# antoyang/FrozenBiLM

Hardware: AMD Instinct MI355X
Metric: video-text samples/sec (MLM fwd+bwd) DeBERTa-XL+adapters (higher is better)
Workload: dtype bf16; 1 GPU; DeBERTa-v2-XLarge(24L)+adapters ds8/8, B=32/GPU, T=10x1024, L=256 (S=266), MLM fwd+bwd+allreduce+clip+Adam, dropout 0.1 live, seeded random weights; global_batch=32, seq_len=266, parallelism=dp1, dead_layer23_encoder_pass=skipped (output unused, SURVEY fact 6); FLOPs still counted

## Files before the change

frozenbilm_amd/bert_engine.py:

```python
from __future__ import annotations

import math
from dataclasses import dataclass
from typing import Dict, List, Optional

import torch

from . import lib as L
from .engine import BF16, F32, Engine, NormRef, Packing, Run, Stream, _ru, _StepFn


@dataclass
class BertLayerSave:
    qkv: torch.Tensor
    ctx: torch.Tensor
    lse: torch.Tensor
    gp: torch.Tensor
    ln1: NormRef
    ln2: NormRef
    seed_att: int
    seed_ln1: int
    seed_ln2: int


# ... 25 lines not shown
    offs = [0]
    for v in plen_h:
        offs.append(offs[-1] + v)
    row0 = torch.tensor(offs, dtype=torch.int32, device=dev)
    b_of = torch.repeat_interleave(torch.arange(B, device=dev), torch.tensor(plen_h, device=dev), output_size=n)
    pos = torch.arange(n, device=dev) - row0[:-1].long()[b_of]
    sel = b_of * S + pos
    inv = torch.full((B * S,), -1, dtype=torch.int64, device=dev)
    inv[sel] = torch.arange(n, device=dev)
    return Packing(row0=row0, sel=sel, inv=inv, pos=pos, n=n)


class BertEngine:
    _ln = Engine._ln
    _ln_bwd = Engine._ln_bwd
    _materialize = Engine._materialize
    attach_grads = Engine.attach_grads

    def __init__(self, model):
        self.m = model
        cfg = model.config
        self.cfg = cfg
        self.H, self.I, self.V = cfg.hidden_size, cfg.intermediate_size, cfg.vocab_size
        self.nh, self.nL = cfg.num_attention_heads, cfg.num_hidden_layers
        if self.H != 64 * self.nh or self.H % 64 or self.I % 64:
            raise NotImplementedError(f"the fused attention takes head_dim 64 (hidden {self.H}, {self.nh} heads) and the GEMMs "
                                      "need hidden / intermediate sizes that are multiples of 64")
        self.F = model.features_dim
        self.Fp = _ru(self.F, 64) if self.F else 0
        self.Vp = _ru(self.V, 64)
# ... 403 lines not shown
```

frozenbilm_amd/build.py:

```python
from __future__ import annotations

import concurrent.futures as cf
import os
import shutil
import subprocess
import sys

HERE = os.path.dirname(os.path.abspath(__file__))
CSRC = os.path.join(HERE, "csrc")
DEBUG = os.environ.get("FBL_DEBUG_BUILD", "0") == "1"
OBJ = os.path.join(HERE, "csrc", "build_dbg" if DEBUG else "build")
LIB = os.path.join(HERE, "libfbl_dbg.so" if DEBUG else "libfbl.so")
ARCH = "gfx950"
FLAGS = ["--offload-arch=" + ARCH, "-O3", "-std=c++17", "-fPIC", "-fno-gpu-rdc", "-Wno-unused-result"]
if DEBUG:
    FLAGS.append("-DFBL_DEBUG_SWITCHES")
    FLAGS += os.environ.get("FBL_DEBUG_EXTRA_FLAGS", "").split()
    if os.environ.get("FBL_DEBUG_LIB_NAME"):
        LIB = os.path.join(HERE, os.environ["FBL_DEBUG_LIB_NAME"])
        OBJ = os.path.join(HERE, "csrc", "build_dbg_" + os.path.splitext(os.environ["FBL_DEBUG_LIB_NAME"])[0])


def _hipcc() -> str:
    for cand in (os.environ.get("HIPCC"), shutil.which("hipcc"), "/opt/rocm/bin/hipcc"):
        if cand and os.path.exists(cand):
            return cand
    raise RuntimeError("hipcc not found (need ROCm >= 7.0 with gfx950 support)")


def sources():
    return sorted(os.path.join(CSRC, f) for f in os.listdir(CSRC) if f.endswith(".hip"))


def _deps_mtime() -> float:
    hdrs = [os.path.join(CSRC, f) for f in os.listdir(CSRC) if f.endswith(".h")]
    hdrs += [os.path.join(os.path.dirname(HERE), "include", h) for h in ("fbl.h", "fbl_mha.h")]
    return max(os.path.getmtime(h) for h in hdrs)


def _compile(src: str, force: bool) -> str:
    obj = os.path.join(OBJ, os.path.basename(src)[:-4] + ".o")
    if not force and os.path.exists(obj) and os.path.getmtime(obj) > max(os.path.getmtime(src), _deps_mtime()):
        return obj
    cmd = [_hipcc(), *FLAGS, "-Rpass-analysis=kernel-resource-usage", "-c", src, "-o", obj]
    r = subprocess.run(cmd, capture_output=True, text=True)
    if r.returncode != 0:
        raise RuntimeError(f"hipcc failed for {src}:\n{r.stdout}\n{r.stderr}")
    bad, name = [], "?"
    for line in r.stderr.splitlines():
        if "Function Name:" in line:
            name = line.split("Function Name:")[1].split("[")[0].strip()
# ... 33 lines not shown
```

frozenbilm_amd/csrc/rowops.hip:

```cpp
#include "fbl_common.h"
#include "../../include/fbl.h"

namespace {

template <int VEC>
struct VecF {};
template <>
struct VecF<4> {
  typedef f32x4 T;
};
template <>
struct VecF<2> {
  typedef f32x2 T;
};

template <int VEC>
__device__ __forceinline__ void ldf(const float* p, float* v) {
  if (VEC == 4) {
    f32x4 x = *(const f32x4*)p;
    v[0] = x[0]; v[1] = x[1]; v[2] = x[2]; v[3] = x[3];
  } else if (VEC == 2) {
    f32x2 x = *(const f32x2*)p;
    v[0] = x[0]; v[1] = x[1];
  } else {
// ... 11 lines not shown
  if (VEC == 4) *(bf16x4*)p = (bf16x4){f2bf(v[0]), f2bf(v[1]), f2bf(v[2]), f2bf(v[3])};
  else if (VEC == 2) *(bf16x2*)p = (bf16x2){f2bf(v[0]), f2bf(v[1])};
  else p[0] = f2bf(v[0]);
}

struct LnFwdArgs {
  const float* y; long ldy; float p_drop; uint64_t seed; const uint64_t* seed_dev;
  const float* r_plain; const float* r_t; const float* r_stats; const float* r_gamma; const float* r_beta;
  const int32_t* r_rowmask;
  const float* gamma; const float* beta; float eps; const int32_t* rowmask;
  float* out_t; float* out_stats; bf16* out_bf16; float* out_f32;
  int N, H;
};

template <int EPL>
__global__ __launch_bounds__(256) void ln_fwd_kernel(LnFwdArgs a) {
  constexpr int VEC = (EPL % 4 == 0) ? 4 : ((EPL % 2 == 0) ? 2 : 1);
  constexpr int NIT = EPL / VEC;
  const int lane = threadIdx.x & 63;
  const int row = blockIdx.x * 4 + (threadIdx.x >> 6);
  if (row >= a.N) return;
  const int H = a.H;
  float v[EPL];
  const uint32_t thr = fbl_drop_thresh(a.p_drop);
  const float inv_keep = a.p_drop > 0.f ? 1.0f / (1.0f - a.p_drop) : 1.0f;
  const uint64_t seed = a.p_drop > 0.f ? fbl_seed(a.seed, a.seed_dev) : 0;
  float rmean = 0.f, rrstd = 0.f, rmask = 1.f;
  if (a.r_t) {
    rmean = a.r_stats[2 * (long)row];
    rrstd = a.r_stats[2 * (long)row + 1];
    if (a.r_rowmask) rmask = (float)a.r_rowmask[row];
  }
#pragma unroll
  for (int it = 0; it < NIT; ++it) {
    const int col = (it * 64 + lane) * VEC;
    float* vv = v + it * VEC;
// ... 38 lines not shown
  if (lane == 0 && a.out_stats) {
    a.out_stats[2 * (long)row] = mean;
    a.out_stats[2 * (long)row + 1] = rstd;
  }
  const float om = a.rowmask ? (float)a.rowmask[row] : 1.0f;
#pragma unroll
  for (int it = 0; it < NIT; ++it) {
    const int col = (it * 64 + lane) * VEC;
    float gg[VEC], bb[VEC], o[VEC];
    ldf<VEC>(a.gamma + col, gg);
    ldf<VEC>(a.beta + col, bb);
#pragma unroll
    for (int c = 0; c < VEC; ++c) o[c] = ((v[it * VEC + c] - mean) * rstd * gg[c] + bb[c]) * om;
    if (a.out_bf16) stb<VEC>(a.out_bf16 + (long)row * H + col, o);
    if (a.out_f32) stf<VEC>(a.out_f32 + (long)row * H + col, o);
  }
}

struct LnMatArgs {
  const float* t; const float* stats; const float* gamma; const float* beta; const int32_t* rowmask;
  const float* add_bcast; int S; float* out_f32; bf16* out_bf16; int N, H;
};
template <int EPL>
__global__ __launch_bounds__(256) void ln_mat_kernel(LnMatArgs a) {
  constexpr int VEC = (EPL % 4 == 0) ? 4 : ((EPL % 2 == 0) ? 2 : 1);
  constexpr int NIT = EPL / VEC;
  const int lane = threadIdx.x & 63;
  const int row = blockIdx.x * 4 + (threadIdx.x >> 6);
  if (row >= a.N) return;
  const int H = a.H;
// ... 711 lines not shown
  return 0;
}

extern "C" int fbl_ln_materialize(const float* t, const float* stats, const float* gamma, const float* beta,
                                  const int32_t* rowmask, const float* add_bcast, int S, float* out_f32, void* out_bf16,
                                  int N, int H, void* stream) {
  if (H % 64 || H > 2048) return FBL_ERR_SHAPE;
  if (N <= 0) return 0;
  LnMatArgs a{t, stats, gamma, beta, rowmask, add_bcast, S > 0 ? S : 1, out_f32, (bf16*)out_bf16, N, H};
  dim3 grid((N + 3) / 4);
  FBL_EPL_DISPATCH(H, ln_mat_kernel, grid, a, (hipStream_t)stream);
  FBL_CHECK_LAUNCH();
  return 0;
}

extern "C" int64_t fbl_ln_bwd_ws_floats(int H) { return (int64_t)LNB_BLOCKS * 3 * H; }
extern "C" int fbl_ln_bwd(const float* dout, const int32_t* rowmask, const float* t, const float* stats,
                          const float* gamma, float p_drop, uint64_t seed, const uint64_t* seed_dev, float* out_dt, void* out_dy_bf16,
                          float* out_dy_f32, float* dgamma, float* dbeta, float* dysum, float* ws, int N, int H,
                          int64_t ld_dy_bf16, void* stream) {
  if (H % 64 || H > 2048) return FBL_ERR_SHAPE;
  if (N <= 0) return 0;
  if (ld_dy_bf16 == 0) ld_dy_bf16 = H;
  if (ld_dy_bf16 < H || (ld_dy_bf16 % 8)) return FBL_ERR_ALIGN;
  LnBwdArgs a{dout, rowmask, t, stats, gamma, p_drop, seed, seed_dev, out_dt, (bf16*)out_dy_bf16, out_dy_f32, ws, N, H, ld_dy_bf16};
  int nblk;
  if ((H / 64) % 2 == 0) {
    nblk = (N + 1) / 2;
    if (nblk > LNB_BLOCKS) nblk = LNB_BLOCKS;
    dim3 grid(nblk);
    switch (H / 64) {
      case 2: hipLaunchKernelGGL(ln_bwd2_kernel<2>, grid, dim3(256), 0, (hipStream_t)stream, a); break;
      case 4: hipLaunchKernelGGL(ln_bwd2_kernel<4>, grid, dim3(256), 0, (hipStream_t)stream, a); break;
      case 8: hipLaunchKernelGGL(ln_bwd2_kernel<8>, grid, dim3(256), 0, (hipStream_t)stream, a); break;
      case 12: hipLaunchKernelGGL(ln_bwd2_kernel<12>, grid, dim3(256), 0, (hipStream_t)stream, a); break;
      case 16: hipLaunchKernelGGL(ln_bwd2_kernel<16>, grid, dim3(256), 0, (hipStream_t)stream, a); break;
      case 24: hipLaunchKernelGGL(ln_bwd2_kernel<24>, grid, dim3(256), 0, (hipStream_t)stream, a); break;
      case 32: hipLaunchKernelGGL(ln_bwd2_kernel<32>, grid, dim3(256), 0, (hipStream_t)stream, a); break;
      default: return FBL_ERR_SHAPE;
    }
  } else {
    nblk = (N + 3) / 4;
    if (nblk > LNB_BLOCKS) nblk = LNB_BLOCKS;
    dim3 grid(nblk);
    FBL_EPL_DISPATCH(H, ln_bwd_kernel, grid, a, (hipStream_t)stream);
  }
  FBL_CHECK_LAUNCH();
  if (dgamma || dbeta || dysum) {
    hipLaunchKernelGGL(ln_bwd_fold_kernel, dim3((3 * H + 31) / 32), dim3(256), 0, (hipStream_t)stream, ws, nblk, H,
                       dgamma, dbeta, dysum);
    FBL_CHECK_LAUNCH();
  }
  return 0;
}

extern "C" int fbl_im2col3(const void* x_bf16, void* out_bf16, int B, int S, int H, void* stream) {
  if (H % 8) return FBL_ERR_SHAPE;
  if (B * S <= 0) return 0;
  hipLaunchKernelGGL(im2col3_kernel, dim3(B * S), dim3(256), 0, (hipStream_t)stream, (const bf16*)x_bf16,
                     (bf16*)out_bf16, B, S, H);
  FBL_CHECK_LAUNCH();
  return 0;
}
extern "C" int fbl_col2im3(const float* dcol, float* dx, int B, int S, int H, int accumulate, void* stream) {
  if (H % 4) return FBL_ERR_SHAPE;
  if (B * S <= 0) return 0;
  hipLaunchKernelGGL(col2im3_kernel, dim3(B * S), dim3(256), 0, (hipStream_t)stream, dcol, dx, B, S, H, accumulate);
// ... 203 lines not shown
```

frozenbilm_amd/engine.py:

```python
from __future__ import annotations

import math
from dataclasses import dataclass, field
from typing import Dict, List, Optional

import numpy as np
import torch

from . import lib as L
from .model.relpos import rel_index_vector

BF16, F32 = torch.bfloat16, torch.float32


def _ru(x: int, m: int) -> int:
    return (x + m - 1) // m * m


@dataclass
class NormRef:
    t: torch.Tensor
    stats: torch.Tensor
    gamma: torch.Tensor
    beta: torch.Tensor
    rowmask: Optional[torch.Tensor] = None

    def as_args(self):
        return (self.t, self.stats, self.gamma, self.beta, self.rowmask)


@dataclass
class Stream:
    bf16: torch.Tensor
    norm: Optional[NormRef] = None
    plain: Optional[torch.Tensor] = None
    full: Optional[torch.Tensor] = None


@dataclass
class Packing:
    row0: torch.Tensor
    sel: torch.Tensor
    inv: torch.Tensor
    pos: torch.Tensor
    n: int


@dataclass
class MergedPack:
    A: int
    WT: torch.Tensor
# ... 32 lines not shown
        self.nL = cfg.num_hidden_layers
        self.span2 = 2 * cfg.att_span
        self.lin_span = min(cfg.position_buckets // 2, cfg.att_span) if cfg.position_buckets > 0 else 0
        self.F = model.features_dim
        self.Fp = _ru(self.F, 64) if self.F else 0
        self.A1 = self.H // model.ds_factor_attn if model.ds_factor_attn else 0
        self.A2 = self.H // model.ds_factor_ff if model.ds_factor_ff else 0
        self.Vp = _ru(self.V, 64)
        dev = model.device
        if dev.type != "cuda":
            raise RuntimeError("frozenbilm_amd runs on MI355X only: move the model to a cuda (HIP) device; "
                               "there is no CPU fallback")
        L.load()
        self.dev = dev
        o = dict(getattr(model, "engine_options", None) or {})
        unknown = set(o) - {"eager_logits", "dw_group", "attn_save_p"}
        if unknown:
            raise ValueError(f"unknown engine_options: {sorted(unknown)}")
        self.eager_logits = bool(o.get("eager_logits", False))
        self.attn_save_p = bool(o.get("attn_save_p", True))
        self.dw_group = max(1, min(L.ADW_MAX_ADAPTERS, int(o.get("dw_group", 16))))
        self._build_flat()
        self._pack_frozen()
        self._build_trainable_operands()
        self._compose_ev = None
        self._relidx: Dict[int, torch.Tensor] = {}
        self._pos_cache: Dict[int, torch.Tensor] = {}
        self._no_pos_cache = False
        self.reducer = None
        self._dyz_pool: Dict[tuple, list] = {}
        self._dyz_shape = None
        self.params_version = 0
        self._ops_version = None
        self.skip_dead_layer = True
        self._ln_ws = L.ln_bwd_ws(self.H, dev)
        self._cs_ws = L.colsum_ws(max(self.H, self.I), dev)
        self.sk_ws = torch.empty(48 << 20, dtype=F32, device=dev)
        self.side = torch.cuda.Stream(device=dev)
        self.side_ws = torch.empty(8 << 20, dtype=F32, device=dev)
        self.side_cs_ws = L.colsum_ws(max(self.H, self.I), dev)
        if L._AUX.get(dev.index if dev.index is not None else torch.cuda.current_device()) is None:
            L.set_aux_stream(torch.cuda.Stream(device=dev), dev)
        L.exclude_from_aux(self.side)

    def _build_flat(self):
        from .model.deberta import flat_order

        m = self.m
        named = dict(m.named_parameters())
        train_names = [n for n, p in named.items() if p.requires_grad]
# ... 340 lines not shown
        inv = torch.full((B * S,), -1, dtype=torch.int64, device=dev)
        inv[sel] = torch.arange(n, device=dev)
        return Packing(row0=row0, sel=sel, inv=inv, pos=pos, n=n)

    def _ln(self, run, name, *, y, resid: Optional[Stream], N, p_drop=0.0, rowmask=None, want_f32=False, tail=0):
        H = self.H
        g, b = self.P[name + ".weight"], self.P[name + ".bias"]
        t = torch.empty(N, H, dtype=F32, device=self.dev)
        stats = torch.empty(N, 2, dtype=F32, device=self.dev)
        full = torch.empty(N + tail, H, dtype=BF16, device=self.dev)
        ob = full[:N]
        of = torch.empty(N, H, dtype=F32, device=self.dev) if want_f32 else None
        seed = run.next_seed() if p_drop > 0 else 0
        r_norm = resid.norm.as_args() if resid is not None and resid.norm is not None else None
        r_plain = resid.plain if resid is not None and r_norm is None else None
        L.ln_fwd(y=y, p_drop=p_drop, seed=seed, r_plain=r_plain, r_norm=r_norm,
                 gamma=g, beta=b, eps=self.cfg.layer_norm_eps, rowmask=rowmask, out_t=t, out_stats=stats, out_bf16=ob,
                 out_f32=of, N=N, H=H)
        return Stream(bf16=ob, norm=NormRef(t, stats, g, b, rowmask), plain=of, full=full if tail else None), seed

    def _adapter_fwd(self, run, site: AdapterSite, x_f32, x_bf16, N):
        A, Ap = site.A, site.Ap
        z = torch.zeros(N, Ap, dtype=BF16, device=self.dev) if Ap != A else torch.empty(N, Ap, dtype=BF16, device=self.dev)
        seed = run.next_seed() if run.p_ad > 0 else 0
        L.adapter_down_fwd(x_bf16, site.down, site.bd, z, A=A, p_drop=run.p_ad, seed=seed)
        y = torch.empty(N, self.H, dtype=F32, device=self.dev)
        L.gemm(z, site.up, bias=site.bu, aux=x_f32, aux_kind=L.AUX_ADD_F32, out_f32=y)
        return y, z, seed

    def _dense_adapter_ln(self, run, li, x_bf16, W, bias, site: Optional[AdapterSite], N, ln_name, resid: Stream, tail=0):
        H, dev = self.H, self.dev
        ob = torch.empty(N, H, dtype=BF16, device=dev)
        if site is None or not site.merged:
            y = torch.empty(N, H, dtype=F32, device=dev)
# ... 5 lines not shown
            return out, ob, z, seed_ad, seed_ln
        if self._compose_ev is not None:
            torch.cuda.current_stream().wait_event(self._compose_ev[0 if li == 0 else 1])
        A = site.A
        z = torch.empty(N, A, dtype=BF16, device=dev)
        seed_ad = run.next_seed() if run.p_ad > 0 else 0
        L.dense_adapter_down_fwd(x_bf16, site.WM, site.bM, H, z, y_bf16=ob, p_drop=run.p_ad, seed=seed_ad)
        g, b = self.P[ln_name + ".weight"], self.P[ln_name + ".bias"]
        t = torch.empty(N, H, dtype=F32, device=dev)
        stats = torch.empty(N, 2, dtype=F32, device=dev)
        full = torch.empty(N + tail, H, dtype=BF16, device=dev)
        seed_ln = run.next_seed() if run.p_hid > 0 else 0
        r_norm = resid.norm.as_args() if resid.norm is not None else None
        L.adapter_up_resid_fwd(z, site.up, site.bu, ob, t, A=A, p_drop=run.p_hid, seed=seed_ln,
                               r_plain=resid.plain if r_norm is None else None, r_norm=r_norm)
        L.ln_fwd(y=t, gamma=g, beta=b, eps=self.cfg.layer_norm_eps, out_stats=stats, out_bf16=full[:N], N=N, H=H)
        return (Stream(bf16=full[:N], norm=NormRef(t, stats, g, b, None), full=full if tail else None), ob, z, seed_ad,
                seed_ln)

    def _pos_proj_cached(self, li: int, W, Rb: torch.Tensor) -> torch.Tensor:
        c = self._pos_cache.get(li)
        if c is None:
            c = torch.empty(self.span2, 2 * self.H, dtype=BF16, device=self.dev)
            L.gemm(Rb, W["Wqkv"][: 2 * self.H], bias=W["bqkv"][: 2 * self.H], out_bf16=c)
            self._pos_cache[li] = c
        return c

    def _layer_fwd(self, run, li: int, kv: Stream, q: Optional[Stream], Rb: torch.Tensor):
        W = self.Lw[li]
        B, S, H, I, nh = run.B, run.S, self.H, self.I, self.nh
        N = run.N
        Sp = _ru(S, 64)
        dev = self.dev
        sv = LayerSave(li=li, emd=q is not None)
        P_ = self.span2
        if run.p_hid > 0:
            sv.seed_pos = run.next_seed()

        def put_r(full):
            if run.p_hid > 0:
                L.dropout_f32(run.R32, run.p_hid, sv.seed_pos, out_bf16=full[N:])
            else:
                full[N:].copy_(Rb)

        infer = not run.save and run.p_hid == 0
        pqk_c = (self._pos_proj_cached(li, W, Rb)
                 if infer and getattr(self.m, "_weights_frozen", 0) > 0 and not self._no_pos_cache else None)
        reuse = infer and q is not None and run.emd_qkv is not None
        if reuse:
            qkv = run.emd_qkv
            if pqk_c is None:
                put_r(q.full)
            L.gemm(q.full if pqk_c is None else q.bf16, W["Wqkv"][:H], bias=W["bqkv"][:H], out_bf16=qkv[:, :H])
        else:
            rows_in = N if pqk_c is not None else N + P_
            qkv = torch.empty(rows_in, 3 * H, dtype=BF16, device=dev)
            kin = kv.full[:rows_in]
            if pqk_c is None:
                put_r(kv.full)
            if q is None:
                L.gemm(kin, W["Wqkv"], bias=W["bqkv"], out_bf16=qkv)
            else:
                if pqk_c is None:
                    put_r(q.full)
                L.gemm(q.full[:rows_in], W["Wqkv"][:H], bias=W["bqkv"][:H], out_bf16=qkv[:, :H])
                L.gemm(kin, W["Wqkv"][H:], bias=W["bqkv"][H:], out_bf16=qkv[:, H:])
                if infer:
                    run.emd_qkv = qkv
        if pqk_c is not None:
            pq, pk = pqk_c[:, :H], pqk_c[:, H:]
        else:
            pq, pk = qkv[N:, :H], qkv[N:, H:2 * H]
        ctx = torch.empty(N, H, dtype=BF16, device=dev)
        lse = torch.empty(B, nh, S, dtype=F32, device=dev)
        sv.seed_att = run.next_seed() if run.p_att > 0 else 0
        psave = msave = None
        if run.save and self.attn_save_p:
            psave = torch.empty(B, nh, Sp, Sp, dtype=BF16, device=dev)
            msave = torch.empty(B, nh, Sp // 64, S, dtype=F32, device=dev)
# ... 203 lines not shown
        L.gemm(col, self.Wc, bias=self.bc, rowscale=run.mask_f, out_f32=c)
        y = torch.empty(N, H, dtype=F32, device=dev)
        run.seed_conv = run.next_seed() if run.p_hid > 0 else 0
        L.dropout_gelu_fwd(c, run.p_hid, run.seed_conv, y)
        out, _ = self._ln(run, "deberta.encoder.conv.LayerNorm", y=y, resid=l0, N=N, rowmask=run.rowmask, tail=self.span2)
        run.conv_c, run.conv_norm = c, out.norm
        return out

    def _ln_bwd(self, name, dout, norm: NormRef, p_drop, seed, want_dy_bf16=True, dysum=None, tail=0, dy_out=None):
        N, H = dout.shape
        dt_full = torch.empty(N + tail, H, dtype=F32, device=self.dev)
        dt = dt_full[:N]
        if tail:
            dt_full[N:].zero_()
        dyb = dy_out if dy_out is not None else (torch.empty(N, H, dtype=BF16, device=self.dev) if want_dy_bf16 else None)
        L.ln_bwd(dout, norm.t, norm.stats, norm.gamma, rowmask=norm.rowmask, p_drop=p_drop, seed=seed, out_dt=dt,
                 out_dy_bf16=dyb, dgamma=self.G.get(name + ".weight"), dbeta=self.G.get(name + ".bias"), dysum=dysum,
                 ws=self._ln_ws)
        if tail:
            return dt, dyb, dt_full
        return dt, dyb

    def _adapter_bwd(self, run, site: AdapterSite, dyb, z, xin_b, seed, dz_out=None, pooled=None):
        N, H = dyb.shape
        A, Ap = site.A, site.Ap
        dev = self.dev
        upT, downT = self._adapter_bwd_operands(site)
        if dz_out is not None:
            dz = dz_out
        else:
            dz = torch.zeros(N, Ap, dtype=BF16, device=dev) if Ap != A else torch.empty(N, Ap, dtype=BF16, device=dev)
        inv_keep = 1.0 / (1.0 - run.p_ad) if run.p_ad > 0 else 1.0
        L.gemm(dyb, upT, alpha=inv_keep, aux=z, aux_kind=L.AUX_MUL_POS_BF16, out_bf16=dz, N=A)
# ... 249 lines not shown
                 dgamma=self.G.get("deberta.embeddings.LayerNorm.weight"), dbeta=self.G.get("deberta.embeddings.LayerNorm.bias"),
                 ws=self._ln_ws)
        if T:
            if pk is None:
                dv = dt0.view(B, S, H)[:, :T].reshape(B * T, H).contiguous()
            else:
                dv = dt0.index_select(0, (pk.row0[:-1].long()[:, None] + torch.arange(T, device=dev)[None]).reshape(-1))
            Kp = _ru(B * T, 64)
            dvT = torch.empty(H, Kp, dtype=BF16, device=dev)
            vT = torch.empty(self.Fp, Kp, dtype=BF16, device=dev)
            L.transpose_to_bf16(dv, dvT)
            L.transpose_to_bf16(run.video_bf16, vT)
            L.gemm(dvT, vT, aux=self.G["deberta.embeddings.linear_video.weight"], aux_kind=L.AUX_ADD_F32,
                   out_f32=self.G["deberta.embeddings.linear_video.weight"], N=self.F)
            L.colsum(dv, self.G["deberta.embeddings.linear_video.bias"], self._cs_ws)
        if red:
            red.ready("emb")
            red.finish()

    def _conv_bwd(self, run, dout):
        B, S, H, dev = run.B, run.S, self.H, self.dev
        N = run.N
        cn = run.conv_norm
        dt = torch.empty(N, H, dtype=F32, device=dev)
        L.ln_bwd(dout, cn.t, cn.stats, cn.gamma, rowmask=cn.rowmask, out_dt=dt,
                 dgamma=self.G.get("deberta.encoder.conv.LayerNorm.weight"),
                 dbeta=self.G.get("deberta.encoder.conv.LayerNorm.bias"), ws=self._ln_ws)
        dc = torch.empty(N, H, dtype=BF16, device=dev)
        L.dropout_gelu_bwd(dt, run.conv_c, run.p_hid, run.seed_conv, out_bf16=dc)
        dcol = torch.empty(N, 3 * H, dtype=F32, device=dev)
        L.gemm(dc, self.WcT, rowscale=run.mask_f, out_f32=dcol)
        return dt, dcol


class _Ready:

    __slots__ = ("eng", "run", "reducer")

    def __init__(self, eng, run, reducer):
        self.eng, self.run, self.reducer = eng, run, reducer

    def ready(self, key):
        if self.run.dw_event is not None:
            torch.cuda.current_stream().wait_event(self.run.dw_event)
        self.reducer.ready(key)

    def finish(self):
        self.reducer.finish()


@dataclass
class LayerSave:
    li: int = 0
    emd: bool = False
    qkv: torch.Tensor = None
    pqk: torch.Tensor = None
    ctx: torch.Tensor = None
# ... 74 lines not shown
    dw_ready_keys: list = field(default_factory=list)
    dw_count: int = 0
    side_used: bool = False
    dw_event: Optional[torch.cuda.Event] = None
    _pos_keep: list = field(default_factory=list)
    pos_chain: Optional["PosChain"] = None

    def __post_init__(self):
        if not self.N:
            self.N = self.B * self.S

    def next_seed(self) -> int:
        self._site += 1
        return (self.seed_base + self._site * 0x85EBCA77) & 0xFFFFFFFFFFFFFFFF


class _StepFn(torch.autograd.Function):

    @staticmethod
    def forward(ctx, engine, run, loss_t, logits_t, *params):
        ctx.engine, ctx.run = engine, run
        ctx.set_materialize_grads(False)
        return loss_t.detach().clone(), logits_t.detach()

    @staticmethod
    def backward(ctx, gloss, glogits):
        eng, run = ctx.engine, ctx.run
        if gloss is not None or glogits is not None:
            eng.backward(run, gloss, glogits)
        return (None, None, None, None) + tuple(None for _ in eng.order)
# ... 1 lines not shown
```

frozenbilm_amd/lib.py:

```python
from __future__ import annotations

import ctypes as C
import os
from typing import Optional

import torch

HERE = os.path.dirname(os.path.abspath(__file__))
LIB_PATH = os.environ.get("FBL_LIB") or os.path.join(HERE, "libfbl.so")

ACT_NONE, ACT_GELU, ACT_RELU, ACT_GELU_GRAD = 0, 1, 2, 3
AUX_NONE, AUX_ADD_F32, AUX_ADD_BF16, AUX_MUL_DGELU_BF16, AUX_MUL_POS_BF16, AUX_MUL_BF16 = 0, 1, 2, 3, 4, 5
ABI_VERSION = 9

_vp, _i, _l, _f, _u64 = C.c_void_p, C.c_int, C.c_int64, C.c_float, C.c_uint64

SIGNATURES = {
    "fbl_abi_version": (_i, []),
    "fbl_gemm_bf16_nt": (_i, [_vp, _l, _vp, _l, _i, _i, _i, _vp, _vp, _f, _i, _i, _vp, _l, _vp, _vp, _vp, _l, _i, _l, _l,
                              _l, _l, _l, _i, _vp, _l, _vp, _vp]),
    "fbl_adapter_down_fwd": (_i, [_vp, _l, _vp, _l, _i, _i, _i, _vp, _f, _u64, _vp, _vp, _l, _vp]),
    "fbl_dense_adapter_down_fwd": (_i, [_vp, _l, _vp, _l, _i, _i, _i, _i, _vp, _vp, _vp, _l, _f, _u64, _vp, _vp, _l, _vp, _vp]),
    "fbl_adapter_up_resid_fwd": (_i, [_vp, _l, _vp, _l, _i, _i, _i, _vp, _vp, _l, _f, _u64, _vp, _vp, _l, _vp, _vp, _vp, _vp,
                                      _vp, _l, _vp]),
# ... 42 lines not shown
    "fbl_dropout_bf16": (_i, [_vp, _f, _u64, _vp, _l, _vp]),
    "fbl_dropout_sum_f32": (_i, [_vp, _l, _l, _i, _vp, _f, _vp, _vp, _vp]),
    "fbl_zero": (_i, [_vp, _l, _vp]),
    "fbl_heads_to_rows_bf16": (_i, [_vp, _vp, _i, _i, _i, _l, _vp]),
}

MHA_SIGNATURES = {
    "fbl_mha_fwd": (_i, [_vp, _l, _vp, _l, _vp, _l, _vp, _vp, _vp, _f, _f, _u64, _vp, _vp, _l, _vp, _i, _i, _i, _vp]),
    "fbl_mha_bwd": (_i, [_vp, _l, _vp, _l, _vp, _l, _vp, _l, _vp, _vp, _vp, _vp, _vp, _f, _f, _u64, _vp, _vp, _l, _vp, _l, _vp, _l,
                         _i, _i, _i, _vp]),
    "fbl_mha_fwd_rows": (_i, [_vp, _l, _vp, _l, _vp, _l, _vp, _vp, _vp, _vp, _f, _f, _u64, _vp, _vp, _l, _vp, _i, _i, _i, _vp]),
    "fbl_mha_bwd_rows": (_i, [_vp, _l, _vp, _l, _vp, _l, _vp, _l, _vp, _l, _vp, _vp, _vp, _vp, _vp, _vp, _f, _f, _u64, _vp, _vp, _l,
                              _vp, _l, _vp, _l, _i, _i, _i, _vp]),
}

_LIB = None


def load(path: Optional[str] = None):
    global _LIB
    if _LIB is not None and path is None:
        return _LIB
    p = path or LIB_PATH
    if not os.path.exists(p):
        raise RuntimeError(
            f"{p} not found: the FrozenBiLM MI355X path needs its HIP library (python -m frozenbilm_amd.build); "
            "there is no CPU/eager fallback")
    lib = C.CDLL(p)
    for name, (res, args) in (*SIGNATURES.items(), *MHA_SIGNATURES.items()):
        fn = getattr(lib, name)
        fn.restype = res
        fn.argtypes = args
    ver = lib.fbl_abi_version()
    if ver != ABI_VERSION:
        raise RuntimeError(f"{p} has ABI version {ver}, this binding needs {ABI_VERSION}: rebuild it "
                           "(python -m frozenbilm_amd.build --force)")
    if path is None:
        _LIB = lib
    return lib


def _p(t: Optional[torch.Tensor]):
    return None if t is None else t.data_ptr()

# ... 266 lines not shown
    ldy = 0
    if y is not None:
        _req(y, torch.float32, "y")
        ldy = _rows2d(y, "y")
    rt = rs = rg = rb = rm = None
    if r_norm is not None:
        rt, rs, rg, rb, rm = r_norm
    for t in (r_plain, rt, out_t, out_bf16, out_f32):
        if t is not None:
            assert t.is_contiguous()
    _chk(load().fbl_ln_fwd(_p(y), ldy, float(p_drop), int(seed), _seed_dev(), _p(r_plain), _p(rt), _p(rs), _p(rg), _p(rb), _p(rm),
                           _p(gamma), _p(beta), float(eps), _p(rowmask), _p(out_t), _p(out_stats), _p(out_bf16),
                           _p(out_f32), N, H, _stream()), "fbl_ln_fwd")


def ln_materialize(t, stats, gamma, beta, rowmask=None, add_bcast=None, S=1, out_f32=None, out_bf16=None):
    N, H = t.shape
    _chk(load().fbl_ln_materialize(_p(t), _p(stats), _p(gamma), _p(beta), _p(rowmask), _p(add_bcast), S, _p(out_f32),
                                   _p(out_bf16), N, H, _stream()), "fbl_ln_materialize")


def ln_bwd_ws(H, device):
    return torch.empty(load().fbl_ln_bwd_ws_floats(H), dtype=torch.float32, device=device)


def ln_bwd(dout, t, stats, gamma, *, rowmask=None, p_drop=0.0, seed=0, out_dt=None, out_dy_bf16=None, out_dy_f32=None,
           dgamma=None, dbeta=None, dysum=None, ws=None):
    N, H = t.shape
    assert dout.is_contiguous() and t.is_contiguous()
    ld_dyb = _rows2d(out_dy_bf16, "out_dy_bf16") if out_dy_bf16 is not None else 0
    _chk(load().fbl_ln_bwd(_p(dout), _p(rowmask), _p(t), _p(stats), _p(gamma), float(p_drop), int(seed), _seed_dev(), _p(out_dt),
                           _p(out_dy_bf16), _p(out_dy_f32), _p(dgamma), _p(dbeta), _p(dysum), _p(ws), N, H, ld_dyb,
                           _stream()), "fbl_ln_bwd")


def im2col3(x_bf16, out_bf16, B, S, H):
    _chk(load().fbl_im2col3(_p(x_bf16), _p(out_bf16), B, S, H, _stream()), "fbl_im2col3")


def col2im3(dcol, dx, B, S, H, accumulate):
    _chk(load().fbl_col2im3(_p(dcol), _p(dx), B, S, H, int(accumulate), _stream()), "fbl_col2im3")


def dropout_gelu_fwd(c, p_drop, seed, out_f32):
    _chk(load().fbl_dropout_gelu_fwd(_p(c), float(p_drop), int(seed), _seed_dev(), _p(out_f32), c.numel(), _stream()),
         "fbl_dropout_gelu_fwd")


# ... 334 lines not shown
```

Baseline: 799.4 samples/s.

## Fuse relative-position dropout tail into LayerNorm forward and defer LN-backward folds to aux stream

The LayerNorm forward kernel gains a tail-block mode that also writes the dropped-out relative-position rows into the same output buffer. This removes the separate dropout_f32 launch before each attention QKV GEMM; it relies on peeking the next seed so the later put_r call can skip its work. In backward, the LN dgamma/dbeta fold kernel moves to an auxiliary stream using a double-buffered workspace and events, with joins before reducer readiness. This takes the fold off the critical path, at the cost of extra event synchronisation and a dependence on the seed peek matching the actual seed.

```diff
diff --git a/frozenbilm_amd/bert_engine.py b/frozenbilm_amd/bert_engine.py
--- a/frozenbilm_amd/bert_engine.py
+++ b/frozenbilm_amd/bert_engine.py
@@ -63,6 +63,8 @@
 class BertEngine:
     _ln = Engine._ln
     _ln_bwd = Engine._ln_bwd
+    _tail_seed = Engine._tail_seed
+    rowop_fusions = False
     _materialize = Engine._materialize
     attach_grads = Engine.attach_grads
 
diff --git a/frozenbilm_amd/build.py b/frozenbilm_amd/build.py
--- a/frozenbilm_amd/build.py
+++ b/frozenbilm_amd/build.py
@@ -34,7 +34,7 @@
 
 def _deps_mtime() -> float:
     hdrs = [os.path.join(CSRC, f) for f in os.listdir(CSRC) if f.endswith(".h")]
-    hdrs += [os.path.join(os.path.dirname(HERE), "include", h) for h in ("fbl.h", "fbl_mha.h")]
+    hdrs += [os.path.join(os.path.dirname(HERE), "include", h) for h in ("fbl.h", "fbl_mha.h", "fbl_rowfuse.h")]
     return max(os.path.getmtime(h) for h in hdrs)
 
 
diff --git a/frozenbilm_amd/csrc/rowops.hip b/frozenbilm_amd/csrc/rowops.hip
--- a/frozenbilm_amd/csrc/rowops.hip
+++ b/frozenbilm_amd/csrc/rowops.hip
@@ -1,5 +1,6 @@
 #include "fbl_common.h"
 #include "../../include/fbl.h"
+#include "../../include/fbl_rowfuse.h"
 
 namespace {
 
@@ -49,12 +50,9 @@
 };
 
 template <int EPL>
-__global__ __launch_bounds__(256) void ln_fwd_kernel(LnFwdArgs a) {
+__device__ __forceinline__ void ln_fwd_row(const LnFwdArgs& a, const int row, const int lane) {
   constexpr int VEC = (EPL % 4 == 0) ? 4 : ((EPL % 2 == 0) ? 2 : 1);
   constexpr int NIT = EPL / VEC;
-  const int lane = threadIdx.x & 63;
-  const int row = blockIdx.x * 4 + (threadIdx.x >> 6);
-  if (row >= a.N) return;
   const int H = a.H;
   float v[EPL];
   const uint32_t thr = fbl_drop_thresh(a.p_drop);
@@ -123,6 +121,46 @@
     for (int c = 0; c < VEC; ++c) o[c] = ((v[it * VEC + c] - mean) * rstd * gg[c] + bb[c]) * om;
     if (a.out_bf16) stb<VEC>(a.out_bf16 + (long)row * H + col, o);
     if (a.out_f32) stf<VEC>(a.out_f32 + (long)row * H + col, o);
+  }
+}
+template <int EPL>
+__global__ __launch_bounds__(256) void ln_fwd_kernel(LnFwdArgs a) {
+  const int row = blockIdx.x * 4 + (threadIdx.x >> 6);
+  if (row >= a.N) return;
+  ln_fwd_row<EPL>(a, row, threadIdx.x & 63);
+}
+
+struct LnFwdTailArgs {
+  LnFwdArgs ln;
+  const float* tail_src; int tail_rows; float tail_p; uint64_t tail_seed;
+};
+template <int EPL>
+__global__ __launch_bounds__(256) void ln_fwd_tail_kernel(LnFwdTailArgs t) {
+  constexpr int VEC = (EPL % 4 == 0) ? 4 : ((EPL % 2 == 0) ? 2 : 1);
+  constexpr int NIT = EPL / VEC;
+  const int lane = threadIdx.x & 63, wave = threadIdx.x >> 6;
+  const int nrb = (t.ln.N + 3) / 4;
+  if ((int)blockIdx.x < nrb) {
+    const int row = blockIdx.x * 4 + wave;
+    if (row < t.ln.N) ln_fwd_row<EPL>(t.ln, row, lane);
+    return;
+  }
+  const int r = ((int)blockIdx.x - nrb) * 4 + wave;
+  if (r >= t.tail_rows) return;
+  const int H = t.ln.H;
+  const uint64_t seed = t.tail_p > 0.f ? fbl_seed(t.tail_seed, t.ln.seed_dev) : 0;
+  const uint32_t thr = fbl_drop_thresh(t.tail_p);
+  const float ik = t.tail_p > 0.f ? 1.f / (1.f - t.tail_p) : 1.f;
+#pragma unroll
+  for (int it = 0; it < NIT; ++it) {
+    const int col = (it * 64 + lane) * VEC;
+    float v[VEC];
+    ldf<VEC>(t.tail_src + (long)r * H + col, v);
+    if (t.tail_p > 0.f) {
+#pragma unroll
+      for (int c = 0; c < VEC; ++c) v[c] *= fbl_dropout_scale(seed, (uint64_t)r * H + col + c, thr, ik);
+    }
+    stb<VEC>(t.ln.out_bf16 + ((long)t.ln.N + r) * H + col, v);
   }
 }
 
@@ -864,7 +902,57 @@
   return 0;
 }
 
+extern "C" int fbl_ln_fwd_tail(const float* y, int64_t ldy, float p_drop, uint64_t seed, const uint64_t* seed_dev,
+                               const float* r_plain, const float* r_t, const float* r_stats, const float* r_gamma,
+                               const float* r_beta, const int32_t* r_rowmask, const float* gamma, const float* beta, float eps,
+                               const int32_t* rowmask, float* out_t, float* out_stats, void* out_bf16, float* out_f32, int N,
+                               int H, const float* tail_src, int tail_rows, float tail_p, uint64_t tail_seed, void* stream) {
+  if (H % 64 || H > 2048) return FBL_ERR_SHAPE;
+  if (r_t && (!r_stats || !r_gamma || !r_beta)) return FBL_ERR_ARG;
+  if (N < 0) N = 0;
+  if (tail_rows < 0) tail_rows = 0;
+  if (tail_rows && (!tail_src || !out_bf16 || tail_p < 0.f || tail_p >= 1.f)) return FBL_ERR_ARG;
+  if (N + tail_rows == 0) return 0;
+  LnFwdTailArgs a{{y, ldy, p_drop, seed, seed_dev, r_plain, r_t, r_stats, r_gamma, r_beta, r_rowmask, gamma, beta, eps, rowmask,
+                   out_t, out_stats, (bf16*)out_bf16, out_f32, N, H},
+                  tail_src, tail_rows, tail_p, tail_seed};
+  dim3 grid((N + 3) / 4 + (tail_rows + 3) / 4);
+  FBL_EPL_DISPATCH(H, ln_fwd_tail_kernel, grid, a, (hipStream_t)stream);
+  FBL_CHECK_LAUNCH();
+  return 0;
+}
+
 extern "C" int64_t fbl_ln_bwd_ws_floats(int H) { return (int64_t)LNB_BLOCKS * 3 * H; }
+extern "C" int64_t fbl_ln_bwd_ws2_floats(int H) { return 2 * fbl_ln_bwd_ws_floats(H); }
+
+static int ln_bwd_rows(const LnBwdArgs& a, int* nblk_out, hipStream_t stream) {
+  const int N = a.N, H = a.H;
+  int nblk;
+  if ((H / 64) % 2 == 0) {
+    nblk = (N + 1) / 2;
+    if (nblk > LNB_BLOCKS) nblk = LNB_BLOCKS;
+    dim3 grid(nblk);
+    switch (H / 64) {
+      case 2: hipLaunchKernelGGL(ln_bwd2_kernel<2>, grid, dim3(256), 0, stream, a); break;
+      case 4: hipLaunchKernelGGL(ln_bwd2_kernel<4>, grid, dim3(256), 0, stream, a); break;
+      case 8: hipLaunchKernelGGL(ln_bwd2_kernel<8>, grid, dim3(256), 0, stream, a); break;
+      case 12: hipLaunchKernelGGL(ln_bwd2_kernel<12>, grid, dim3(256), 0, stream, a); break;
+      case 16: hipLaunchKernelGGL(ln_bwd2_kernel<16>, grid, dim3(256), 0, stream, a); break;
+      case 24: hipLaunchKernelGGL(ln_bwd2_kernel<24>, grid, dim3(256), 0, stream, a); break;
+      case 32: hipLaunchKernelGGL(ln_bwd2_kernel<32>, grid, dim3(256), 0, stream, a); break;
+      default: return FBL_ERR_SHAPE;
+    }
+  } else {
+    nblk = (N + 3) / 4;
+    if (nblk > LNB_BLOCKS) nblk = LNB_BLOCKS;
+    dim3 grid(nblk);
+    FBL_EPL_DISPATCH(H, ln_bwd_kernel, grid, a, stream);
+  }
+  FBL_CHECK_LAUNCH();
+  *nblk_out = nblk;
+  return 0;
+}
+
 extern "C" int fbl_ln_bwd(const float* dout, const int32_t* rowmask, const float* t, const float* stats,
                           const float* gamma, float p_drop, uint64_t seed, const uint64_t* seed_dev, float* out_dt, void* out_dy_bf16,
                           float* out_dy_f32, float* dgamma, float* dbeta, float* dysum, float* ws, int N, int H,
@@ -875,32 +963,86 @@
   if (ld_dy_bf16 < H || (ld_dy_bf16 % 8)) return FBL_ERR_ALIGN;
   LnBwdArgs a{dout, rowmask, t, stats, gamma, p_drop, seed, seed_dev, out_dt, (bf16*)out_dy_bf16, out_dy_f32, ws, N, H, ld_dy_bf16};
   int nblk;
-  if ((H / 64) % 2 == 0) {
-    nblk = (N + 1) / 2;
-    if (nblk > LNB_BLOCKS) nblk = LNB_BLOCKS;
-    dim3 grid(nblk);
-    switch (H / 64) {
-      case 2: hipLaunchKernelGGL(ln_bwd2_kernel<2>, grid, dim3(256), 0, (hipStream_t)stream, a); break;
-      case 4: hipLaunchKernelGGL(ln_bwd2_kernel<4>, grid, dim3(256), 0, (hipStream_t)stream, a); break;
-      case 8: hipLaunchKernelGGL(ln_bwd2_kernel<8>, grid, dim3(256), 0, (hipStream_t)stream, a); break;
-      case 12: hipLaunchKernelGGL(ln_bwd2_kernel<12>, grid, dim3(256), 0, (hipStream_t)stream, a); break;
-      case 16: hipLaunchKernelGGL(ln_bwd2_kernel<16>, grid, dim3(256), 0, (hipStream_t)stream, a); break;
-      case 24: hipLaunchKernelGGL(ln_bwd2_kernel<24>, grid, dim3(256), 0, (hipStream_t)stream, a); break;
-      case 32: hipLaunchKernelGGL(ln_bwd2_kernel<32>, grid, dim3(256), 0, (hipStream_t)stream, a); break;
-      default: return FBL_ERR_SHAPE;
-    }
-  } else {
-    nblk = (N + 3) / 4;
-    if (nblk > LNB_BLOCKS) nblk = LNB_BLOCKS;
-    dim3 grid(nblk);
-    FBL_EPL_DISPATCH(H, ln_bwd_kernel, grid, a, (hipStream_t)stream);
-  }
-  FBL_CHECK_LAUNCH();
+  if (const int rc = ln_bwd_rows(a, &nblk, (hipStream_t)stream)) return rc;
   if (dgamma || dbeta || dysum) {
     hipLaunchKernelGGL(ln_bwd_fold_kernel, dim3((3 * H + 31) / 32), dim3(256), 0, (hipStream_t)stream, ws, nblk, H,
                        dgamma, dbeta, dysum);
     FBL_CHECK_LAUNCH();
   }
+  return 0;
+}
+
+#include <map>
+#include <mutex>
+namespace {
+struct LnDefer {
+  hipEvent_t fork = nullptr, done[2] = {nullptr, nullptr};
+  bool pending[2] = {false, false};
+  int next = 0, last = 0;
+};
+std::mutex ln_defer_mu;
+std::map<hipStream_t, LnDefer> ln_defer_pool;
+LnDefer* ln_defer_state(hipStream_t s, bool create) {
+  auto it = ln_defer_pool.find(s);
+  if (it != ln_defer_pool.end()) return &it->second;
+  if (!create) return nullptr;
+  LnDefer d;
+  if (hipEventCreateWithFlags(&d.fork, hipEventDisableTiming) != hipSuccess) return nullptr;
+  for (int h = 0; h < 2; ++h)
+    if (hipEventCreateWithFlags(&d.done[h], hipEventDisableTiming) != hipSuccess) return nullptr;
+  return &ln_defer_pool.emplace(s, d).first->second;
+}
+}
+
+extern "C" int fbl_ln_bwd_deferred(const float* dout, const int32_t* rowmask, const float* t, const float* stats,
+                                   const float* gamma, float p_drop, uint64_t seed, const uint64_t* seed_dev, float* out_dt,
+                                   void* out_dy_bf16, float* out_dy_f32, float* dgamma, float* dbeta, float* dysum, float* ws2,
+                                   int N, int H, int64_t ld_dy_bf16, void* stream, void* aux_stream) {
+  if (H % 64 || H > 2048) return FBL_ERR_SHAPE;
+  if (N <= 0) return 0;
+  if (ld_dy_bf16 == 0) ld_dy_bf16 = H;
+  if (ld_dy_bf16 < H || (ld_dy_bf16 % 8)) return FBL_ERR_ALIGN;
+  if (!ws2) return FBL_ERR_ARG;
+  const hipStream_t s = (hipStream_t)stream, aux = (hipStream_t)aux_stream;
+  std::lock_guard<std::mutex> lock(ln_defer_mu);
+  LnDefer* d = ln_defer_state(s, true);
+  if (!d) return FBL_ERR_ARG;
+  const int h = d->next;
+  d->next ^= 1;
+  if (d->pending[h]) {
+    if (hipStreamWaitEvent(s, d->done[h], 0) != hipSuccess) return FBL_ERR_ARG;
+    d->pending[h] = false;
+  }
+  float* ws = ws2 + (int64_t)h * fbl_ln_bwd_ws_floats(H);
+  LnBwdArgs a{dout, rowmask, t, stats, gamma, p_drop, seed, seed_dev, out_dt, (bf16*)out_dy_bf16, out_dy_f32, ws, N, H, ld_dy_bf16};
+  int nblk;
+  if (const int rc = ln_bwd_rows(a, &nblk, s)) return rc;
+  if (!(dgamma || dbeta || dysum)) return 0;
+  const bool defer = aux && aux != s;
+  if (defer) {
+    if (hipEventRecord(d->fork, s) != hipSuccess) return FBL_ERR_ARG;
+    if (hipStreamWaitEvent(aux, d->fork, 0) != hipSuccess) return FBL_ERR_ARG;
+  } else if (d->pending[h ^ 1]) {
+    if (hipStreamWaitEvent(s, d->done[h ^ 1], 0) != hipSuccess) return FBL_ERR_ARG;
+    d->pending[h ^ 1] = false;
+  }
+  hipLaunchKernelGGL(ln_bwd_fold_kernel, dim3((3 * H + 31) / 32), dim3(256), 0, defer ? aux : s, ws, nblk, H, dgamma, dbeta,
+                     dysum);
+  FBL_CHECK_LAUNCH();
+  if (defer) {
+    if (hipEventRecord(d->done[h], aux) != hipSuccess) return FBL_ERR_ARG;
+    d->pending[h] = true;
+    d->last = h;
+  }
+  return 0;
+}
+
+extern "C" int fbl_ln_bwd_join(void* stream) {
+  std::lock_guard<std::mutex> lock(ln_defer_mu);
+  LnDefer* d = ln_defer_state((hipStream_t)stream, false);
+  if (!d || !(d->pending[0] || d->pending[1])) return 0;
+  if (hipStreamWaitEvent((hipStream_t)stream, d->done[d->last], 0) != hipSuccess) return FBL_ERR_ARG;
+  d->pending[0] = d->pending[1] = false;
   return 0;
 }
 
diff --git a/frozenbilm_amd/engine.py b/frozenbilm_amd/engine.py
--- a/frozenbilm_amd/engine.py
+++ b/frozenbilm_amd/engine.py
@@ -35,6 +35,7 @@
     norm: Optional[NormRef] = None
     plain: Optional[torch.Tensor] = None
     full: Optional[torch.Tensor] = None
+    tail_seed: Optional[int] = None
 
 
 @dataclass
@@ -97,7 +98,7 @@
         L.load()
         self.dev = dev
         o = dict(getattr(model, "engine_options", None) or {})
-        unknown = set(o) - {"eager_logits", "dw_group", "attn_save_p"}
+        unknown = set(o) - {"eager_logits", "dw_group", "attn_save_p", "rowop_fusions"}
         if unknown:
             raise ValueError(f"unknown engine_options: {sorted(unknown)}")
         self.eager_logits = bool(o.get("eager_logits", False))
@@ -117,6 +118,8 @@
         self._ops_version = None
         self.skip_dead_layer = True
         self._ln_ws = L.ln_bwd_ws(self.H, dev)
+        self.rowop_fusions = bool(o.get("rowop_fusions", True))
+        self._ln_ws2 = L.ln_bwd_ws2(self.H, dev)
         self._cs_ws = L.colsum_ws(max(self.H, self.I), dev)
         self.sk_ws = torch.empty(48 << 20, dtype=F32, device=dev)
         self.side = torch.cuda.Stream(device=dev)
@@ -487,10 +490,23 @@
         seed = run.next_seed() if p_drop > 0 else 0
         r_norm = resid.norm.as_args() if resid is not None and resid.norm is not None else None
         r_plain = resid.plain if resid is not None and r_norm is None else None
-        L.ln_fwd(y=y, p_drop=p_drop, seed=seed, r_plain=r_plain, r_norm=r_norm,
-                 gamma=g, beta=b, eps=self.cfg.layer_norm_eps, rowmask=rowmask, out_t=t, out_stats=stats, out_bf16=ob,
-                 out_f32=of, N=N, H=H)
-        return Stream(bf16=ob, norm=NormRef(t, stats, g, b, rowmask), plain=of, full=full if tail else None), seed
+        tail_seed = self._tail_seed(run, tail)
+        if tail_seed is not None:
+            L.ln_fwd_tail(y=y, p_drop=p_drop, seed=seed, r_plain=r_plain, r_norm=r_norm,
+                          gamma=g, beta=b, eps=self.cfg.layer_norm_eps, rowmask=rowmask, out_t=t, out_stats=stats, out_bf16=full,
+                          out_f32=of, N=N, H=H, tail_src=run.R32, tail_p=run.p_hid, tail_seed=tail_seed)
+        else:
+            L.ln_fwd(y=y, p_drop=p_drop, seed=seed, r_plain=r_plain, r_norm=r_norm,
+                     gamma=g, beta=b, eps=self.cfg.layer_norm_eps, rowmask=rowmask, out_t=t, out_stats=stats, out_bf16=ob,
+                     out_f32=of, N=N, H=H)
+        return Stream(bf16=ob, norm=NormRef(t, stats, g, b, rowmask), plain=of, full=full if tail else None,
+                      tail_seed=tail_seed), seed
+
+    def _tail_seed(self, run, tail) -> Optional[int]:
+        if not (tail and self.rowop_fusions and run.p_hid > 0 and run.R32 is not None):
+            return None
+        assert tail == run.R32.shape[0]
+        return run.peek_seed()
 
     def _adapter_fwd(self, run, site: AdapterSite, x_f32, x_bf16, N):
         A, Ap = site.A, site.Ap
@@ -526,9 +542,14 @@
         r_norm = resid.norm.as_args() if resid.norm is not None else None
         L.adapter_up_resid_fwd(z, site.up, site.bu, ob, t, A=A, p_drop=run.p_hid, seed=seed_ln,
                                r_plain=resid.plain if r_norm is None else None, r_norm=r_norm)
-        L.ln_fwd(y=t, gamma=g, beta=b, eps=self.cfg.layer_norm_eps, out_stats=stats, out_bf16=full[:N], N=N, H=H)
-        return (Stream(bf16=full[:N], norm=NormRef(t, stats, g, b, None), full=full if tail else None), ob, z, seed_ad,
-                seed_ln)
+        tail_seed = self._tail_seed(run, tail)
+        if tail_seed is not None:
+            L.ln_fwd_tail(y=t, gamma=g, beta=b, eps=self.cfg.layer_norm_eps, out_stats=stats, out_bf16=full, N=N, H=H,
+                          tail_src=run.R32, tail_p=run.p_hid, tail_seed=tail_seed)
+        else:
+            L.ln_fwd(y=t, gamma=g, beta=b, eps=self.cfg.layer_norm_eps, out_stats=stats, out_bf16=full[:N], N=N, H=H)
+        return (Stream(bf16=full[:N], norm=NormRef(t, stats, g, b, None), full=full if tail else None, tail_seed=tail_seed),
+                ob, z, seed_ad, seed_ln)
 
     def _pos_proj_cached(self, li: int, W, Rb: torch.Tensor) -> torch.Tensor:
         c = self._pos_cache.get(li)
@@ -549,8 +570,11 @@
         if run.p_hid > 0:
             sv.seed_pos = run.next_seed()
 
-        def put_r(full):
+        def put_r(st: Stream):
+            full = st.full
             if run.p_hid > 0:
+                if st.tail_seed == sv.seed_pos:
+                    return
                 L.dropout_f32(run.R32, run.p_hid, sv.seed_pos, out_bf16=full[N:])
             else:
                 full[N:].copy_(Rb)
@@ -562,19 +586,19 @@
         if reuse:
             qkv = run.emd_qkv
             if pqk_c is None:
-                put_r(q.full)
+                put_r(q)
             L.gemm(q.full if pqk_c is None else q.bf16, W["Wqkv"][:H], bias=W["bqkv"][:H], out_bf16=qkv[:, :H])
         else:
             rows_in = N if pqk_c is not None else N + P_
             qkv = torch.empty(rows_in, 3 * H, dtype=BF16, device=dev)
             kin = kv.full[:rows_in]
             if pqk_c is None:
-                put_r(kv.full)
+                put_r(kv)
             if q is None:
                 L.gemm(kin, W["Wqkv"], bias=W["bqkv"], out_bf16=qkv)
             else:
                 if pqk_c is None:
-                    put_r(q.full)
+                    put_r(q)
                 L.gemm(q.full[:rows_in], W["Wqkv"][:H], bias=W["bqkv"][:H], out_bf16=qkv[:, :H])
                 L.gemm(kin, W["Wqkv"][H:], bias=W["bqkv"][H:], out_bf16=qkv[:, H:])
                 if infer:
@@ -808,9 +832,14 @@
         if tail:
             dt_full[N:].zero_()
         dyb = dy_out if dy_out is not None else (torch.empty(N, H, dtype=BF16, device=self.dev) if want_dy_bf16 else None)
-        L.ln_bwd(dout, norm.t, norm.stats, norm.gamma, rowmask=norm.rowmask, p_drop=p_drop, seed=seed, out_dt=dt,
-                 out_dy_bf16=dyb, dgamma=self.G.get(name + ".weight"), dbeta=self.G.get(name + ".bias"), dysum=dysum,
-                 ws=self._ln_ws)
+        if self.rowop_fusions:
+            L.ln_bwd_deferred(dout, norm.t, norm.stats, norm.gamma, rowmask=norm.rowmask, p_drop=p_drop, seed=seed, out_dt=dt,
+                              out_dy_bf16=dyb, dgamma=self.G.get(name + ".weight"), dbeta=self.G.get(name + ".bias"),
+                              dysum=dysum, ws2=self._ln_ws2)
+        else:
+            L.ln_bwd(dout, norm.t, norm.stats, norm.gamma, rowmask=norm.rowmask, p_drop=p_drop, seed=seed, out_dt=dt,
+                     out_dy_bf16=dyb, dgamma=self.G.get(name + ".weight"), dbeta=self.G.get(name + ".bias"), dysum=dysum,
+                     ws=self._ln_ws)
         if tail:
             return dt, dyb, dt_full
         return dt, dyb
@@ -1090,6 +1119,7 @@
             L.gemm(dvT, vT, aux=self.G["deberta.embeddings.linear_video.weight"], aux_kind=L.AUX_ADD_F32,
                    out_f32=self.G["deberta.embeddings.linear_video.weight"], N=self.F)
             L.colsum(dv, self.G["deberta.embeddings.linear_video.bias"], self._cs_ws)
+        L.ln_bwd_join()
         if red:
             red.ready("emb")
             red.finish()
@@ -1117,6 +1147,7 @@
         self.eng, self.run, self.reducer = eng, run, reducer
 
     def ready(self, key):
+        L.ln_bwd_join()
         if self.run.dw_event is not None:
             torch.cuda.current_stream().wait_event(self.run.dw_event)
         self.reducer.ready(key)
@@ -1221,6 +1252,9 @@
         self._site += 1
         return (self.seed_base + self._site * 0x85EBCA77) & 0xFFFFFFFFFFFFFFFF
 
+    def peek_seed(self) -> int:
+        return (self.seed_base + (self._site + 1) * 0x85EBCA77) & 0xFFFFFFFFFFFFFFFF
+
 
 class _StepFn(torch.autograd.Function):
 
diff --git a/frozenbilm_amd/lib.py b/frozenbilm_amd/lib.py
--- a/frozenbilm_amd/lib.py
+++ b/frozenbilm_amd/lib.py
@@ -80,6 +80,14 @@
                               _vp, _l, _vp, _l, _i, _i, _i, _vp]),
 }
 
+ROWFUSE_SIGNATURES = {
+    "fbl_ln_fwd_tail": (_i, [_vp, _l, _f, _u64, _vp, _vp, _vp, _vp, _vp, _vp, _vp, _vp, _vp, _f, _vp, _vp, _vp, _vp, _vp, _i, _i,
+                             _vp, _i, _f, _u64, _vp]),
+    "fbl_ln_bwd_ws2_floats": (_l, [_i]),
+    "fbl_ln_bwd_deferred": (_i, [_vp, _vp, _vp, _vp, _vp, _f, _u64, _vp, _vp, _vp, _vp, _vp, _vp, _vp, _vp, _i, _i, _l, _vp, _vp]),
+    "fbl_ln_bwd_join": (_i, [_vp]),
+}
+
 _LIB = None
 
 
@@ -93,7 +101,7 @@
             f"{p} not found: the FrozenBiLM MI355X path needs its HIP library (python -m frozenbilm_amd.build); "
             "there is no CPU/eager fallback")
     lib = C.CDLL(p)
-    for name, (res, args) in (*SIGNATURES.items(), *MHA_SIGNATURES.items()):
+    for name, (res, args) in (*SIGNATURES.items(), *MHA_SIGNATURES.items(), *ROWFUSE_SIGNATURES.items()):
         fn = getattr(lib, name)
         fn.restype = res
         fn.argtypes = args
@@ -390,6 +398,26 @@
                            _p(out_f32), N, H, _stream()), "fbl_ln_fwd")
 
 
+def ln_fwd_tail(*, y=None, p_drop=0.0, seed=0, r_plain=None, r_norm=None, gamma, beta, eps, rowmask=None, out_t=None,
+                out_stats=None, out_bf16, out_f32=None, N, H, tail_src, tail_p, tail_seed):
+    ldy = 0
+    if y is not None:
+        _req(y, torch.float32, "y")
+        ldy = _rows2d(y, "y")
+    _req(tail_src, torch.float32, "tail_src"); _req(out_bf16, torch.bfloat16, "out_bf16")
+    rt = rs = rg = rb = rm = None
+    if r_norm is not None:
+        rt, rs, rg, rb, rm = r_norm
+    for t in (r_plain, rt, out_t, out_bf16, out_f32, tail_src):
+        if t is not None:
+            assert t.is_contiguous()
+    P = tail_src.shape[0]
+    assert tail_src.shape[1] == H and tuple(out_bf16.shape) == (N + P, H)
+    _chk(load().fbl_ln_fwd_tail(_p(y), ldy, float(p_drop), int(seed), _seed_dev(), _p(r_plain), _p(rt), _p(rs), _p(rg), _p(rb),
+                                _p(rm), _p(gamma), _p(beta), float(eps), _p(rowmask), _p(out_t), _p(out_stats), _p(out_bf16),
+                                _p(out_f32), N, H, _p(tail_src), P, float(tail_p), int(tail_seed), _stream()), "fbl_ln_fwd_tail")
+
+
 def ln_materialize(t, stats, gamma, beta, rowmask=None, add_bcast=None, S=1, out_f32=None, out_bf16=None):
     N, H = t.shape
     _chk(load().fbl_ln_materialize(_p(t), _p(stats), _p(gamma), _p(beta), _p(rowmask), _p(add_bcast), S, _p(out_f32),
@@ -408,6 +436,24 @@
     _chk(load().fbl_ln_bwd(_p(dout), _p(rowmask), _p(t), _p(stats), _p(gamma), float(p_drop), int(seed), _seed_dev(), _p(out_dt),
                            _p(out_dy_bf16), _p(out_dy_f32), _p(dgamma), _p(dbeta), _p(dysum), _p(ws), N, H, ld_dyb,
                            _stream()), "fbl_ln_bwd")
+
+
+def ln_bwd_ws2(H, device):
+    return torch.empty(load().fbl_ln_bwd_ws2_floats(H), dtype=torch.float32, device=device)
+
+
+def ln_bwd_deferred(dout, t, stats, gamma, *, rowmask=None, p_drop=0.0, seed=0, out_dt=None, out_dy_bf16=None, out_dy_f32=None,
+                    dgamma=None, dbeta=None, dysum=None, ws2=None):
+    N, H = t.shape
+    assert dout.is_contiguous() and t.is_contiguous()
+    ld_dyb = _rows2d(out_dy_bf16, "out_dy_bf16") if out_dy_bf16 is not None else 0
+    _chk(load().fbl_ln_bwd_deferred(_p(dout), _p(rowmask), _p(t), _p(stats), _p(gamma), float(p_drop), int(seed), _seed_dev(),
+                                    _p(out_dt), _p(out_dy_bf16), _p(out_dy_f32), _p(dgamma), _p(dbeta), _p(dysum), _p(ws2), N, H,
+                                    ld_dyb, _stream(), _aux_stream()), "fbl_ln_bwd_deferred")
+
+
+def ln_bwd_join():
+    _chk(load().fbl_ln_bwd_join(_stream()), "fbl_ln_bwd_join")
 
 
 def im2col3(x_bf16, out_bf16, B, S, H):
diff --git a/include/fbl_rowfuse.h b/include/fbl_rowfuse.h
--- /dev/null
+++ b/include/fbl_rowfuse.h
@@ -0,0 +1,24 @@
+#ifndef FBL_ROWFUSE_H
+#define FBL_ROWFUSE_H
+#include "fbl.h"
+#ifdef __cplusplus
+extern "C" {
+#endif
+
+int fbl_ln_fwd_tail(const float* y, int64_t ldy, float p_drop, uint64_t seed, const uint64_t* seed_dev, const float* r_plain,
+                    const float* r_t, const float* r_stats, const float* r_gamma, const float* r_beta,
+                    const int32_t* r_rowmask, const float* gamma, const float* beta, float eps, const int32_t* rowmask,
+                    float* out_t, float* out_stats, void* out_bf16, float* out_f32, int N, int H, const float* tail_src,
+                    int tail_rows, float tail_p, uint64_t tail_seed, void* stream);
+
+int64_t fbl_ln_bwd_ws2_floats(int H);
+int fbl_ln_bwd_deferred(const float* dout, const int32_t* rowmask, const float* t, const float* stats, const float* gamma,
+                        float p_drop, uint64_t seed, const uint64_t* seed_dev, float* out_dt, void* out_dy_bf16,
+                        float* out_dy_f32, float* dgamma, float* dbeta, float* dysum, float* ws2, int N, int H,
+                        int64_t ld_dy_bf16, void* stream, void* aux_stream);
+int fbl_ln_bwd_join(void* stream);
+
+#ifdef __cplusplus
+}
+#endif
+#endif
```

New measurement: 799.1 samples/s. No clear change (-0.0%).
